# skypilot-org/skypilot

Hardware: AMD Instinct MI355X
Metric: tokens/sec (node) sky-launched Llama-3-8B (higher is better)
Workload: dtype bf16; 1 GPU; model=llama3-8b, global_batch=6, seq_len=4096, parallelism=dp1, sky_launched=True

## Files before the change

### skypilot_amd/ops/csrc/attention_bwd.hip

```cpp
#include "attn_launch.h"
#include "common.h"

#define BM 64
#define BN 64

extern "C" __global__ void attn_bwd_pre_kernel(
    const unsigned short* __restrict__ dO, const unsigned short* __restrict__ O,
    float* __restrict__ Dvec, long long rows, int S, int Hq) {
  const int lane = threadIdx.x & 63;
  const long long wave_id =
      (long long)blockIdx.x * (blockDim.x >> 6) + (threadIdx.x >> 6);
  const long long stride = (long long)gridDim.x * (blockDim.x >> 6);
  for (long long row = wave_id; row < rows; row += stride) {
    const unsigned short* drow = dO + row * ATT_D;
    const unsigned short* orow = O + row * ATT_D;
    float acc = bf2f(drow[lane]) * bf2f(orow[lane]) +
                bf2f(drow[lane + 64]) * bf2f(orow[lane + 64]);
    acc = wave_reduce_sum(acc);
    const int hh = (int)(row % Hq);
    const long long bs = row / Hq;
    const int ss = (int)(bs % S);
    const long long bb = bs / S;
    if (lane == 0) Dvec[(bb * Hq + hh) * S + ss] = acc;
  }
// ... 219 lines not shown
      *(s16x8*)((char*)v_lds + swz(row * 256 + ch * 16, row)) = vv8;
#pragma unroll
      for (int j = 0; j < 8; ++j) {
        int d = ch * 8 + j;
        *(unsigned short*)((char*)kt_lds + swzT(d * 128 + row * 2, d)) =
            (unsigned short)kv8[j];
      }
    }
    __syncthreads();

    f32x4 st[4], dpt[4];
#pragma unroll
    for (int kv4 = 0; kv4 < 4; ++kv4) {
      st[kv4] = f32x4{0.f, 0.f, 0.f, 0.f};
      dpt[kv4] = f32x4{0.f, 0.f, 0.f, 0.f};
    }
#pragma unroll
    for (int ks = 0; ks < 4; ++ks)
#pragma unroll
      for (int kv4 = 0; kv4 < 4; ++kv4) {
        int krow = kv4 * 16 + lrow;
        s16x8 a_k = *(const s16x8*)((char*)k_lds +
            swz(krow * 256 + (ks * 32 + lgrp * 8) * 2, krow));
        st[kv4] = MFMA_BF16(as_bf16x8(a_k), as_bf16x8(q_b[ks]), st[kv4]);
        s16x8 a_v = *(const s16x8*)((char*)v_lds +
            swz(krow * 256 + (ks * 32 + lgrp * 8) * 2, krow));
        dpt[kv4] = MFMA_BF16(as_bf16x8(a_v), as_bf16x8(do_b[ks]),
                             dpt[kv4]);
      }

#pragma unroll
    for (int kv4 = 0; kv4 < 4; ++kv4)
#pragma unroll
      for (int r = 0; r < 4; ++r) {
        int kv = kvbase + kv4 * 16 + lgrp * 4 + r;
        float pv;
        if ((causal && kv > my_q) || my_lse == -INFINITY)
          pv = 0.f;
        else
          pv = __expf(st[kv4][r] * scale - my_lse);
        st[kv4][r] = pv * (dpt[kv4][r] - my_dvec);
      }

    s16x8 ds_b[2];
#pragma unroll
    for (int ks = 0; ks < 2; ++ks)
#pragma unroll
      for (int j = 0; j < 8; ++j) {
        int src = (2 * (lgrp & 1) + (j >> 2)) * 16 + lrow;
        float v0 = __shfl(st[2 * ks][j & 3], src, 64);
        float v1 = __shfl(st[2 * ks + 1][j & 3], src, 64);
        ds_b[ks][j] = (short)f2bf((lgrp >> 1) ? v1 : v0);
      }

#pragma unroll
    for (int ct = 0; ct < 8; ++ct)
#pragma unroll
      for (int ks = 0; ks < 2; ++ks) {
        int krow = ct * 16 + lrow;
        s16x8 a_kt = *(const s16x8*)((char*)kt_lds +
            swzT(krow * 128 + (ks * 32 + lgrp * 8) * 2, krow));
        dq_t[ct] = MFMA_BF16(as_bf16x8(a_kt), as_bf16x8(ds_b[ks]),
                             dq_t[ct]);
      }
  }

  unsigned short* dQb = dQ + ((long long)b * S * Hq + qh) * ATT_D;
  unsigned short* orow = dQb + (long long)my_q * q_rowstride;
#pragma unroll
  for (int ct = 0; ct < 8; ++ct) {
    s16x4 ov;
#pragma unroll
    for (int r = 0; r < 4; ++r)
      ov[r] = (short)f2bf(dq_t[ct][r] * scale);
    *(s16x4*)(orow + ct * 16 + lgrp * 4) = ov;
  }
}

extern "C" void attn_bwd_launch(const void* Q, const void* K, const void* V,
                                const void* O, const void* dO,
                                const float* lse, float* Dvec, void* dQ,
                                void* dK, void* dV, int B, int S, int Hq,
                                int Hkv, float scale, bool causal,
                                int dkv_variant, hipStream_t stream) {
  long long rows = (long long)B * S * Hq;
  hipLaunchKernelGGL(attn_bwd_pre_kernel, dim3(membound_grid(rows, 4)),
                     dim3(256), 0, stream, (const unsigned short*)dO,
                     (const unsigned short*)O, Dvec, rows, S, Hq);
  if (S % 128 == 0) {
    attn_bwd_v3_launch(Q, K, V, dO, lse, Dvec, dQ, dK, dV, B, S, Hq, Hkv,
                       scale, causal, dkv_variant, stream);
    return;
  }
  hipLaunchKernelGGL(attn_bwd_dkv_kernel, dim3(S / BN, B * Hkv), dim3(256),
                     0, stream, (const unsigned short*)Q,
                     (const unsigned short*)K, (const unsigned short*)V,
                     (const unsigned short*)dO, lse, Dvec,
                     (unsigned short*)dK, (unsigned short*)dV, B, S, Hq, Hkv,
                     scale, causal ? 1 : 0);
  hipLaunchKernelGGL(attn_bwd_dq_swapped_kernel, dim3(S / BM, B * Hq),
                     dim3(256), 0, stream, (const unsigned short*)Q,
                     (const unsigned short*)K, (const unsigned short*)V,
                     (const unsigned short*)dO, lse, Dvec,
                     (unsigned short*)dQ, B, S, Hq, Hkv, scale,
                     causal ? 1 : 0);
}
```

### skypilot_amd/ops/csrc/attention_bwd_v3.hip

```cpp
#include "attn_launch.h"
#include "attn_v3.h"

__device__ __forceinline__ int vsubz(int q, int d) {
  return (((q >> 2) << 3) + ((d >> 4) ^ ((q >> 2) & 7))) * 64 +
         ((q & 3) << 4) + (d & 15);
}

extern "C" __global__ __launch_bounds__(256, 2) void attn_bwd_dkv_v3_kernel(
    const unsigned short* __restrict__ Q, const unsigned short* __restrict__ K,
    const unsigned short* __restrict__ V, const unsigned short* __restrict__ dO,
    const float* __restrict__ lse, const float* __restrict__ Dvec,
    unsigned short* __restrict__ dK, unsigned short* __restrict__ dV, int B,
    int S, int Hq, int Hkv, float scale, int causal) {
  __shared__ unsigned short q_lds[32 * ATT_D];
  __shared__ unsigned short do_lds[32 * ATT_D];
  __shared__ unsigned short k_own[128 * ATT_D];
  __shared__ unsigned short v_own[128 * ATT_D];

  const int kt = blockIdx.x;
  const int bh = blockIdx.y;
  const int b = bh / Hkv;
  const int kvh = bh % Hkv;
  const int group = Hq / Hkv;
  const int kvb = kt * 128;
// ... 564 lines not shown
    for (int n = 0; n < 2; ++n)
#pragma unroll
      for (int r = 0; r < 16; ++r) {
        float p = exp2f(st[n][r] - lse2);
        dpt[n][r] = p * (dpt[n][r] - dvq);
      }

    tr4 t0, t1;
    s16x8 db;
#define DQ_TR_ISSUE(ks)                                                   \
  {                                                                       \
    unsigned base = (unsigned)(size_t)((char*)k_lds[buf]);                \
    int kv_s = (ks) * 16 + ((g >> 1) << 3) + (lw >> 2);                   \
    int d_s0 = ((g & 1) << 4) + ((lw & 3) << 2);                          \
    unsigned a0 = (unsigned)(kv_s * 256 +                                 \
                             ((((d_s0) >> 3) ^ (kv_s & 15)) << 4) +       \
                             ((d_s0 & 7) << 1));                          \
    unsigned a1 = (unsigned)((kv_s + 4) * 256 +                           \
                             ((((d_s0) >> 3) ^ ((kv_s + 4) & 15)) << 4) + \
                             ((d_s0 & 7) << 1));                          \
    unsigned a2 = (unsigned)(kv_s * 256 +                                 \
                             ((((32 + d_s0) >> 3) ^ (kv_s & 15)) << 4) +  \
                             ((d_s0 & 7) << 1));                          \
    unsigned a3 = (unsigned)((kv_s + 4) * 256 +                           \
                             ((((32 + d_s0) >> 3) ^ ((kv_s + 4) & 15))    \
                              << 4) +                                     \
                             ((d_s0 & 7) << 1));                          \
    ds_tr4_issue(&t0, base + a0, base + a1, base + a2, base + a3);        \
    unsigned a4 = (unsigned)(kv_s * 256 +                                 \
                             ((((64 + d_s0) >> 3) ^ (kv_s & 15)) << 4) +  \
                             ((d_s0 & 7) << 1));                          \
    unsigned a5 = (unsigned)((kv_s + 4) * 256 +                           \
                             ((((64 + d_s0) >> 3) ^ ((kv_s + 4) & 15))    \
                              << 4) +                                     \
                             ((d_s0 & 7) << 1));                          \
    unsigned a6 = (unsigned)(kv_s * 256 +                                 \
                             ((((96 + d_s0) >> 3) ^ (kv_s & 15)) << 4) +  \
                             ((d_s0 & 7) << 1));                          \
    unsigned a7 = (unsigned)((kv_s + 4) * 256 +                           \
                             ((((96 + d_s0) >> 3) ^ ((kv_s + 4) & 15))    \
                              << 4) +                                     \
                             ((d_s0 & 7) << 1));                          \
    ds_tr4_issue(&t1, base + a4, base + a5, base + a6, base + a7);        \
  }
#define DQ_MFMA(bfrag)                                                    \
  {                                                                       \
    union { unsigned long long u[2]; s16x8 v; } af;                       \
    __builtin_amdgcn_s_setprio(1);                                        \
    af.u[0] = t0.d[0];                                                    \
    af.u[1] = t0.d[1];                                                    \
    dq_acc[0] = MFMA32V3(as_bf16x8(af.v), as_bf16x8(bfrag), dq_acc[0]);   \
    af.u[0] = t0.d[2];                                                    \
    af.u[1] = t0.d[3];                                                    \
    dq_acc[1] = MFMA32V3(as_bf16x8(af.v), as_bf16x8(bfrag), dq_acc[1]);   \
    af.u[0] = t1.d[0];                                                    \
    af.u[1] = t1.d[1];                                                    \
    dq_acc[2] = MFMA32V3(as_bf16x8(af.v), as_bf16x8(bfrag), dq_acc[2]);   \
    af.u[0] = t1.d[2];                                                    \
    af.u[1] = t1.d[3];                                                    \
    dq_acc[3] = MFMA32V3(as_bf16x8(af.v), as_bf16x8(bfrag), dq_acc[3]);   \
    __builtin_amdgcn_s_setprio(0);                                        \
  }
    DQ_TR_ISSUE(0);
    V3_PACK2(db, dpt, 0);
    lgkm_wait0_bind2(&t0, &t1);
    DQ_MFMA(db);
    DQ_TR_ISSUE(1);
    V3_PACK2(db, dpt, 1);
    lgkm_wait0_bind2(&t0, &t1);
    DQ_MFMA(db);
    DQ_TR_ISSUE(2);
    V3_PACK2(db, dpt, 2);
    lgkm_wait0_bind2(&t0, &t1);
    DQ_MFMA(db);
    DQ_TR_ISSUE(3);
    V3_PACK2(db, dpt, 3);
    lgkm_wait0_bind2(&t0, &t1);
    DQ_MFMA(db);
  }

  DQ_EPILOGUE();
#undef DQ_EPILOGUE
#undef DQ_LOAD_Q
}

extern "C" void attn_bwd_v3_launch(const void* Q, const void* K,
                                   const void* V, const void* dO,
                                   const float* lse, const float* Dvec,
                                   void* dQ, void* dK, void* dV, int B,
                                   int S, int Hq, int Hkv, float scale,
                                   bool causal, int dkv_variant,
                                   hipStream_t stream) {
  const int variant = dkv_variant >= 0 ? dkv_variant : 2;
  if (variant == 0) {
    dim3 gkv(S / 128, B * Hkv);
    hipLaunchKernelGGL(attn_bwd_dkv_v3_kernel, gkv, dim3(256), 0, stream,
                       (const unsigned short*)Q, (const unsigned short*)K,
                       (const unsigned short*)V, (const unsigned short*)dO,
                       lse, Dvec, (unsigned short*)dK, (unsigned short*)dV,
                       B, S, Hq, Hkv, scale, causal ? 1 : 0);
  } else {
    const int heavy_first = variant == 2 ? 1 : 0;
    dim3 gkv = heavy_first ? dim3(B * Hkv, S / 128) : dim3(S / 128, B * Hkv);
    hipLaunchKernelGGL(attn_bwd_dkv_v3p_kernel, gkv, dim3(256), 0, stream,
                       (const unsigned short*)Q, (const unsigned short*)K,
                       (const unsigned short*)V, (const unsigned short*)dO,
                       lse, Dvec, (unsigned short*)dK, (unsigned short*)dV,
                       B, S, Hq, Hkv, scale, causal ? 1 : 0, heavy_first);
  }
  int nqq = S / 128;
  int gqx = (causal && nqq % 2 == 0) ? nqq / 2 : nqq;
  dim3 gq(gqx, B * Hq);
  hipLaunchKernelGGL(attn_bwd_dq_v3_kernel, gq, dim3(256), 0, stream,
                     (const unsigned short*)Q, (const unsigned short*)K,
                     (const unsigned short*)V, (const unsigned short*)dO,
                     lse, Dvec, (unsigned short*)dQ, B, S, Hq, Hkv, scale,
                     causal ? 1 : 0);
}
```

### skypilot_amd/ops/csrc/attn_launch.h

```cpp
#pragma once

#include <hip/hip_runtime.h>

#define ATT_D 128

extern "C" {
void attn_fwd_launch(const void* Q, const void* K, const void* V, void* O,
                     float* lse, int B, int S, int Hq, int Hkv, float scale,
                     bool causal, hipStream_t stream);
void attn_bwd_launch(const void* Q, const void* K, const void* V,
                     const void* O, const void* dO, const float* lse,
                     float* Dvec, void* dQ, void* dK, void* dV, int B, int S,
                     int Hq, int Hkv, float scale, bool causal,
                     int dkv_variant, hipStream_t stream);

void attn_fwd_v3_launch(const void* Q, const void* K, const void* V, void* O,
                        float* lse, int B, int S, int Hq, int Hkv,
                        float scale, bool causal, hipStream_t stream);
void attn_bwd_v3_launch(const void* Q, const void* K, const void* V,
                        const void* dO, const float* lse, const float* Dvec,
                        void* dQ, void* dK, void* dV, int B, int S, int Hq,
                        int Hkv, float scale, bool causal, int dkv_variant,
                        hipStream_t stream);
}
```

### skypilot_amd/ops/csrc/attn_v3.h

```cpp
#pragma once
#include "common.h"

typedef __attribute__((ext_vector_type(16))) float f32x16;
#define MFMA32V3(a, b, c) \
  __builtin_amdgcn_mfma_f32_32x32x16_bf16(a, b, c, 0, 0, 0)

__device__ __forceinline__ int swzK16(int byte_off, int row) {
  return byte_off ^ ((row & 15) << 4);
}

__device__ __forceinline__ int vsub(int kv, int d) {
  return (((kv >> 2) << 3) + (d >> 4)) * 64 + ((kv & 3) << 4) + (d & 15);
}

__device__ __forceinline__ unsigned cvtpk_bf16(float a, float b) {
  unsigned r;
  asm volatile("v_cvt_pk_bf16_f32 %0, %1, %2" : "=v"(r) : "v"(a), "v"(b));
  return r;
}

__device__ __forceinline__ float xhalf32(float x) {
  union { float f; unsigned u; } c;
  c.f = x;
  auto p = __builtin_amdgcn_permlane32_swap(c.u, c.u, false, false);
  union { unsigned u; float f; } r0, r1;
  r0.u = p[0];
  r1.u = p[1];
  return (threadIdx.x & 32) ? r0.f : r1.f;
}

__device__ __forceinline__ void vm_drain() {
  asm volatile("s_waitcnt vmcnt(0)" ::: "memory");
}

__device__ __forceinline__ void lgkm_wait0_bind2(tr4* a, tr4* b) {
  asm volatile("s_waitcnt lgkmcnt(0)"
               : "+v"(a->d[0]), "+v"(a->d[1]), "+v"(a->d[2]),
                 "+v"(a->d[3]), "+v"(b->d[0]), "+v"(b->d[1]),
                 "+v"(b->d[2]), "+v"(b->d[3])
               :
               : "memory");
  __builtin_amdgcn_sched_barrier(0);
}

template <int OFF>
__device__ __forceinline__ void ds_tr4_issue_off(tr4* t, unsigned a0,
                                                 unsigned a1, unsigned a2,
                                                 unsigned a3) {
  static_assert(OFF >= 0 && OFF < 65536, "DS offset field is 16 bits");
  asm volatile(
      "ds_read_b64_tr_b16 %0, %4 offset:%8\n\t"
      "ds_read_b64_tr_b16 %1, %5 offset:%8\n\t"
      "ds_read_b64_tr_b16 %2, %6 offset:%8\n\t"
      "ds_read_b64_tr_b16 %3, %7 offset:%8"
      : "=v"(t->d[0]), "=v"(t->d[1]), "=v"(t->d[2]), "=v"(t->d[3])
      : "v"(a0), "v"(a1), "v"(a2), "v"(a3), "n"(OFF)
      : "memory");
}

__device__ __forceinline__ void gload_lds16(const void* g, void* l) {
  __builtin_amdgcn_global_load_lds(
      (const __attribute__((address_space(1))) unsigned int*)g,
      (__attribute__((address_space(3))) unsigned int*)l, 16, 0, 0);
}


#define V3_PACK_CORE(pb, c0, c1, c2, c3, c4, c5, c6, c7)                  \
  {                                                                       \
    unsigned w0a = cvtpk_bf16(c0, c1);                                    \
    unsigned w1a = cvtpk_bf16(c2, c3);                                    \
    unsigned w0b = cvtpk_bf16(c4, c5);                                    \
    unsigned w1b = cvtpk_bf16(c6, c7);                                    \
    auto p0 = __builtin_amdgcn_permlane32_swap(w0a, w0b, false, false);   \
    auto p1 = __builtin_amdgcn_permlane32_swap(w1a, w1b, false, false);   \
    union { unsigned u[4]; s16x8 v; } pk;                                 \
    pk.u[0] = p0[0];                                                      \
    pk.u[1] = p1[0];                                                      \
    pk.u[2] = p0[1];                                                      \
    pk.u[3] = p1[1];                                                      \
    pb = pk.v;                                                            \
  }
#define V3_PACK2(pb, stv, ks)                                             \
  {                                                                       \
    const int e0 = ((ks) & 1) << 3;                                       \
    const int n = (ks) >> 1;                                              \
    V3_PACK_CORE(pb, stv[n][e0 + 0], stv[n][e0 + 1], stv[n][e0 + 2],      \
                 stv[n][e0 + 3], stv[n][e0 + 4], stv[n][e0 + 5],          \
                 stv[n][e0 + 6], stv[n][e0 + 7]);                         \
  }
#define V3_PACK1(pb, stv, ks)                                             \
  {                                                                       \
    const int e0 = (ks) << 3;                                             \
    V3_PACK_CORE(pb, stv[e0 + 0], stv[e0 + 1], stv[e0 + 2],               \
                 stv[e0 + 3], stv[e0 + 4], stv[e0 + 5], stv[e0 + 6],      \
                 stv[e0 + 7]);                                            \
  }
```

### skypilot_amd/ops/csrc/bindings.cpp

```cpp
#include <torch/extension.h>

#include <ATen/hip/HIPContext.h>
#include <hip/hip_runtime.h>

#include <vector>

#include "attn_append.h"
#include "attn_launch.h"

#define CHECK_GPU(x) TORCH_CHECK(x.is_cuda(), #x " must be on GPU")
#define CHECK_CONTIG(x) TORCH_CHECK(x.is_contiguous(), #x " must be contiguous")
#define CHECK_BF16(x) \
  TORCH_CHECK(x.scalar_type() == at::kBFloat16, #x " must be bf16")

static hipStream_t cur_stream() {
  return at::hip::getCurrentHIPStream().stream();
}

extern "C" {
void rmsnorm_fwd_launch(const void*, const void*, void*, float*, long long,
                        int, float, hipStream_t);
void rmsnorm_bwd_launch(const void*, const void*, const void*, const float*,
                        void*, float*, long long, int, hipStream_t);
void rope_launch(const void*, void*, const float*, const float*, const int*,
// ... 117 lines not shown
              H, D, backward, cur_stream());
  return y;
}

void adamw_step(std::vector<torch::Tensor> params_bf16,
                std::vector<torch::Tensor> params_master,
                std::vector<torch::Tensor> grads,
                std::vector<torch::Tensor> exp_avg,
                std::vector<torch::Tensor> exp_avg_sq, double lr, double beta1,
                double beta2, double eps, double weight_decay, int64_t step,
                double grad_scale, std::vector<bool> decay_mask) {
  auto stream = cur_stream();
  for (size_t i = 0; i < params_bf16.size(); ++i) {
    auto& p = params_bf16[i];
    long long n = p.numel();
    float wd = decay_mask.empty() || decay_mask[i] ? (float)weight_decay : 0.f;
    adamw_launch(p.data_ptr(), params_master[i].data_ptr<float>(),
                 grads[i].data_ptr(), exp_avg[i].data_ptr<float>(),
                 exp_avg_sq[i].data_ptr<float>(), n, (float)lr, (float)beta1,
                 (float)beta2, (float)eps, wd, (int)step, (float)grad_scale,
                 stream);
  }
}

torch::Tensor cross_entropy_fused(torch::Tensor logits, torch::Tensor targets,
                                  double grad_scale, int64_t ignore_index) {
  CHECK_GPU(logits); CHECK_CONTIG(logits); CHECK_BF16(logits);
  TORCH_CHECK(targets.scalar_type() == at::kInt);
  const int V = (int)logits.size(-1);
  long long N = logits.numel() / V;
  auto loss = torch::empty({(long)N}, logits.options().dtype(at::kFloat));
  cross_entropy_launch(logits.data_ptr(), targets.data_ptr<int>(),
                       loss.data_ptr<float>(), N, V, (float)grad_scale,
                       (int)ignore_index, cur_stream());
  return loss;
}

static void check_attn_qkv(const char* op, const torch::Tensor& Q,
                           const torch::Tensor& K, const torch::Tensor& V) {
  const torch::Tensor* ts[] = {&Q, &K, &V};
  const char* names[] = {"Q", "K", "V"};
  for (int i = 0; i < 3; ++i) {
    const torch::Tensor& t = *ts[i];
    TORCH_CHECK(t.is_cuda(), op, ": ", names[i], " must be on GPU");
    TORCH_CHECK(t.scalar_type() == at::kBFloat16, op, ": ", names[i],
                " must be bf16, got ", t.scalar_type());
    TORCH_CHECK(t.dim() == 4, op, ": ", names[i],
                " must be [B, S, heads, 128], got ", t.dim(), " dims");
    TORCH_CHECK(t.is_contiguous(), op, ": ", names[i],
                " must be contiguous, got strides ", t.strides());
    TORCH_CHECK(t.size(3) == ATT_D, op, ": ", names[i],
                " head dim must be 128, got ", t.size(3));
  }
  const int64_t B = Q.size(0), S = Q.size(1), Hq = Q.size(2);
  TORCH_CHECK(S % 64 == 0, op, ": seq len must be a multiple of 64, got ", S);
  TORCH_CHECK(K.size(0) == B && K.size(1) == S, op,
              ": K must be [B, S, Hkv, 128] with Q's B = ", B, " and S = ", S,
              ", got ", K.sizes());
  TORCH_CHECK(V.sizes() == K.sizes(), op, ": V must have K's shape ",
              K.sizes(), ", got ", V.sizes());
  const int64_t Hkv = K.size(2);
  TORCH_CHECK(Hkv > 0 && Hq % Hkv == 0, op, ": Hq = ", Hq,
              " must be a multiple of Hkv = ", Hkv);
}

std::vector<torch::Tensor> attn_fwd(torch::Tensor Q, torch::Tensor K,
                                    torch::Tensor V, double scale,
                                    bool causal) {
  check_attn_qkv("attn_fwd", Q, K, V);
  const int B = (int)Q.size(0), S = (int)Q.size(1), Hq = (int)Q.size(2);
  const int Hkv = (int)K.size(2);
  auto O = torch::empty_like(Q);
  auto lse = torch::empty({B, Hq, S}, Q.options().dtype(at::kFloat));
  attn_fwd_launch(Q.data_ptr(), K.data_ptr(), V.data_ptr(), O.data_ptr(),
                  lse.data_ptr<float>(), B, S, Hq, Hkv, (float)scale, causal,
                  cur_stream());
  return {O, lse};
}

std::vector<torch::Tensor> attn_bwd(torch::Tensor Q, torch::Tensor K,
                                    torch::Tensor V, torch::Tensor O,
                                    torch::Tensor dO, torch::Tensor lse,
                                    double scale, bool causal,
                                    int64_t dkv_variant) {
  check_attn_qkv("attn_bwd", Q, K, V);
  TORCH_CHECK(dkv_variant >= -1 && dkv_variant <= 2,
              "attn_bwd: dkv_variant must be -1, 0, 1 or 2");
  const int B = (int)Q.size(0), S = (int)Q.size(1), Hq = (int)Q.size(2);
  const int Hkv = (int)K.size(2);
  const torch::Tensor* outs[] = {&O, &dO};
  const char* out_names[] = {"O", "dO"};
  for (int i = 0; i < 2; ++i) {
    const torch::Tensor& t = *outs[i];
    TORCH_CHECK(t.is_cuda() && t.scalar_type() == at::kBFloat16, "attn_bwd: ",
                out_names[i], " must be bf16 on GPU, got ", t.scalar_type());
    TORCH_CHECK(t.sizes() == Q.sizes(), "attn_bwd: ", out_names[i],
                " must have Q's shape ", Q.sizes(), ", got ", t.sizes());
    TORCH_CHECK(t.is_contiguous(), "attn_bwd: ", out_names[i],
                " must be contiguous, got strides ", t.strides());
  }
  TORCH_CHECK(lse.is_cuda() && lse.scalar_type() == at::kFloat,
              "attn_bwd: lse must be fp32 on GPU, got ", lse.scalar_type());
  TORCH_CHECK(lse.dim() == 3 && lse.size(0) == B && lse.size(1) == Hq &&
                  lse.size(2) == S,
              "attn_bwd: lse must be [B, Hq, S] = [", B, ", ", Hq, ", ", S,
              "], got ", lse.sizes());
  TORCH_CHECK(lse.is_contiguous(),
              "attn_bwd: lse must be contiguous, got strides ", lse.strides());
  auto dQ = torch::empty_like(Q);
  auto dK = torch::empty_like(K);
  auto dV = torch::empty_like(V);
  auto Dvec = torch::empty({(long)B * S * Hq}, Q.options().dtype(at::kFloat));
  attn_bwd_launch(Q.data_ptr(), K.data_ptr(), V.data_ptr(), O.data_ptr(),
                  dO.data_ptr(), lse.data_ptr<float>(),
                  Dvec.data_ptr<float>(), dQ.data_ptr(), dK.data_ptr(),
                  dV.data_ptr(), B, S, Hq, Hkv, (float)scale, causal,
                  (int)dkv_variant, cur_stream());
  return {dQ, dK, dV};
}

torch::Tensor attn_decode(torch::Tensor Q, torch::Tensor Kc,
                          torch::Tensor Vc, torch::Tensor kv_lens,
                          torch::Tensor slot_ids, double scale) {
  CHECK_GPU(Q); CHECK_CONTIG(Q); CHECK_BF16(Q);
  TORCH_CHECK(kv_lens.scalar_type() == at::kInt);
  TORCH_CHECK(slot_ids.scalar_type() == at::kInt);
  const int B = (int)Q.size(0), Hq = (int)Q.size(1), D = (int)Q.size(2);
  const int S_max = (int)Kc.size(1), Hkv = (int)Kc.size(2);
  TORCH_CHECK(D == 128);
  auto O = torch::empty_like(Q);
  attn_decode_launch(Q.data_ptr(), Kc.data_ptr(), Vc.data_ptr(),
                     O.data_ptr(), kv_lens.data_ptr<int>(),
                     slot_ids.data_ptr<int>(), B, S_max, Hq,
                     Hkv, (float)scale, cur_stream());
  return O;
}

torch::Tensor attn_append(torch::Tensor Q, torch::Tensor Kc,
                          torch::Tensor Vc, torch::Tensor slot_ids,
                          torch::Tensor q_start, torch::Tensor q_lens,
                          double scale) {
  const char* op = "attn_append";
  const torch::Tensor* ts[] = {&Q, &Kc, &Vc};
  const char* names[] = {"Q", "Kc", "Vc"};
  for (int i = 0; i < 3; ++i) {
    const torch::Tensor& t = *ts[i];
    TORCH_CHECK(t.is_cuda(), op, ": ", names[i], " must be on GPU");
    TORCH_CHECK(t.scalar_type() == at::kBFloat16, op, ": ", names[i],
                " must be bf16, got ", t.scalar_type());
    TORCH_CHECK(t.dim() == 4, op, ": ", names[i],
                " must have 4 dims [.., .., heads, 128], got ", t.dim());
    TORCH_CHECK(t.is_contiguous(), op, ": ", names[i],
                " must be contiguous, got strides ", t.strides());
    TORCH_CHECK(t.size(3) == ATT_D, op, ": ", names[i],
                " head dim must be 128, got ", t.size(3));
  }
  const int64_t n = Q.size(0), Sq = Q.size(1), Hq = Q.size(2);
  const int64_t slots = Kc.size(0), S_max = Kc.size(1), Hkv = Kc.size(2);
  TORCH_CHECK(Sq > 0 && Sq % 64 == 0, op,
              ": chunk length Sq must be a positive multiple of 64, got ",
              Sq);
  TORCH_CHECK(Vc.sizes() == Kc.sizes(), op, ": Vc must have Kc's shape ",
              Kc.sizes(), ", got ", Vc.sizes());
  TORCH_CHECK(slots > 0 && S_max > 0, op,
              ": the cache must hold at least one slot and one row, got ",
              Kc.sizes());
  TORCH_CHECK(Hkv > 0 && Hq % Hkv == 0, op, ": Hq = ", Hq,
              " must be a multiple of Hkv = ", Hkv);
  TORCH_CHECK(n > 0 && n * Hq <= 65535, op, ": n * Hq = ", n * Hq,
              " must be in [1, 65535] (one grid row per sequence and head)");
  TORCH_CHECK(Q.device() == Kc.device() && Q.device() == Vc.device(), op,
              ": Q, Kc and Vc must be on one device");
  const torch::Tensor* idx[] = {&slot_ids, &q_start, &q_lens};
  const char* idx_names[] = {"slot_ids", "q_start", "q_lens"};
  for (int i = 0; i < 3; ++i) {
    const torch::Tensor& t = *idx[i];
    TORCH_CHECK(t.is_cuda() && t.device() == Q.device(), op, ": ",
                idx_names[i], " must be on Q's GPU");
    TORCH_CHECK(t.scalar_type() == at::kInt, op, ": ", idx_names[i],
                " must be int32, got ", t.scalar_type());
    TORCH_CHECK(t.dim() == 1 && t.size(0) == n && t.is_contiguous(), op,
                ": ", idx_names[i], " must be a contiguous [n] = [", n,
                "] tensor, got ", t.sizes());
  }
  auto O = torch::empty_like(Q);
  attn_append_launch(Q.data_ptr(), Kc.data_ptr(), Vc.data_ptr(),
                     O.data_ptr(), slot_ids.data_ptr<int>(),
                     q_start.data_ptr<int>(), q_lens.data_ptr<int>(), (int)n,
                     (int)Sq, (int)Hq, (int)Hkv, (int)slots, (int)S_max,
                     (float)scale, cur_stream());
  return O;
}

torch::Tensor attn_decode_qkv(torch::Tensor qkv, torch::Tensor Kc,
                              torch::Tensor Vc, torch::Tensor cos_tab,
                              torch::Tensor sin_tab,
                              torch::Tensor positions,
                              torch::Tensor kv_lens,
                              torch::Tensor slot_ids, int64_t Hq,
                              int64_t Hkv, double scale) {
// ... 244 lines not shown
  TORCH_CHECK(qkv.size(1) == (Hq + 2 * Hkv) * D,
              "rope_kvwrite: packed width mismatch");
  auto q = torch::empty({n, (long)Hq, (long)D}, qkv.options());
  rope_kvwrite_launch(qkv.data_ptr(), q.data_ptr(), kc.data_ptr(),
                      vc.data_ptr(), cos_tab.data_ptr(),
                      sin_tab.data_ptr(), positions.data_ptr(),
                      slot_ids.data_ptr(), n, (int)Hq, (int)Hkv, D, S_max,
                      cur_stream());
  return q;
}

torch::Tensor swiglu_fwd(torch::Tensor gu) {
  CHECK_GPU(gu); CHECK_CONTIG(gu); CHECK_BF16(gu);
  const int M2 = (int)gu.size(-1);
  TORCH_CHECK(M2 % 16 == 0, "swiglu_fwd: last dim must be 2*M with "
              "M % 8 == 0, got ", M2);
  long long rows = gu.numel() / M2;
  auto sizes = gu.sizes().vec();
  sizes.back() = M2 / 2;
  auto y = torch::empty(sizes, gu.options());
  swiglu_fwd_launch(gu.data_ptr(), y.data_ptr(), rows, M2 / 2,
                    cur_stream());
  return y;
}

torch::Tensor swiglu_bwd(torch::Tensor gu, torch::Tensor dy) {
  CHECK_GPU(gu); CHECK_CONTIG(gu); CHECK_BF16(gu);
  CHECK_GPU(dy); CHECK_CONTIG(dy); CHECK_BF16(dy);
  const int M2 = (int)gu.size(-1);
  TORCH_CHECK(M2 % 16 == 0, "swiglu_bwd: last dim must be 2*M with "
              "M % 8 == 0, got ", M2);
  auto ysizes = gu.sizes().vec();
  ysizes.back() = M2 / 2;
  TORCH_CHECK(dy.sizes() == at::IntArrayRef(ysizes),
              "swiglu_bwd: dy must have the shape of swiglu_fwd(gu)");
  long long rows = gu.numel() / M2;
  auto dgu = torch::empty_like(gu);
  swiglu_bwd_launch(gu.data_ptr(), dy.data_ptr(), dgu.data_ptr(), rows,
                    M2 / 2, cur_stream());
  return dgu;
}

torch::Tensor mfma_probe(torch::Tensor A, torch::Tensor B) {
  CHECK_GPU(A); CHECK_BF16(A); CHECK_CONTIG(A); CHECK_CONTIG(B);
  TORCH_CHECK(A.size(0) == 16 && A.size(1) == 32);
  TORCH_CHECK(B.size(0) == 32 && B.size(1) == 16);
  auto C = torch::zeros({16, 16}, A.options().dtype(at::kFloat));
  mfma_probe_launch(A.data_ptr(), B.data_ptr(), C.data_ptr<float>(),
                    cur_stream());
  return C;
}

torch::Tensor mfma32_probe(torch::Tensor A, torch::Tensor B) {
  CHECK_GPU(A); CHECK_BF16(A); CHECK_CONTIG(A); CHECK_CONTIG(B);
  TORCH_CHECK(A.size(0) == 32 && A.size(1) == 16);
  TORCH_CHECK(B.size(0) == 16 && B.size(1) == 32);
  auto C = torch::zeros({32, 32}, A.options().dtype(at::kFloat));
  mfma32_probe_launch(A.data_ptr(), B.data_ptr(), C.data_ptr<float>(),
                      cur_stream());
  return C;
}

torch::Tensor trb16_probe(int64_t mode, torch::Tensor ref_dev) {
  auto out = torch::zeros({64, 4}, ref_dev.options().dtype(at::kFloat));
  trb16_probe_launch(out.data_ptr<float>(), (int)mode, cur_stream());
  return out;
}

torch::Tensor permlane_probe(torch::Tensor ref_dev) {
  auto out = torch::zeros({64, 2}, ref_dev.options().dtype(at::kFloat));
  permlane_probe_launch(out.data_ptr<float>(), cur_stream());
  return out;
}

PYBIND11_MODULE(TORCH_EXTENSION_NAME, m) {
  m.def("rmsnorm_fwd", &rmsnorm_fwd);
  m.def("rmsnorm_bwd", &rmsnorm_bwd);
  m.def("rope", &rope);
  m.def("adamw_step", &adamw_step);
  m.def("cross_entropy_fused", &cross_entropy_fused);
  m.def("attn_fwd", &attn_fwd);
  m.def("attn_bwd", &attn_bwd, py::arg("Q"), py::arg("K"), py::arg("V"),
        py::arg("O"), py::arg("dO"), py::arg("lse"), py::arg("scale"),
        py::arg("causal"), py::arg("dkv_variant") = -1);
  m.def("attn_decode", &attn_decode);
  m.def("attn_append", &attn_append);
  m.def("skinny_gemm", &skinny_gemm);
  m.def("skinny_gemm_fp8", &skinny_gemm_fp8);
  m.def("transpose_bf16", &transpose_bf16);
  m.def("gemm_nt", &gemm_nt);
  m.def("wgrad_tn", &wgrad_tn);
  m.def("adamw_step_mt", &adamw_step_mt);
  m.def("skinny_gemm_swiglu", &skinny_gemm_swiglu);
  m.def("rmsnorm_res", &rmsnorm_res);
  m.def("rope_kvwrite", &rope_kvwrite);
  m.def("decode_advance", &decode_advance);
  m.def("sample_tokens", &sample_tokens);
  m.def("decode_sample_advance", &decode_sample_advance);
  m.def("attn_decode_qkv", &attn_decode_qkv);
  m.def("skinny_gemm_fp8_norm", &skinny_gemm_fp8_norm);
  m.def("swiglu_fwd", &swiglu_fwd);
  m.def("swiglu_bwd", &swiglu_bwd);
  m.def("mfma_probe", &mfma_probe);
  m.def("mfma32_probe", &mfma32_probe);
  m.def("trb16_probe", &trb16_probe);
  m.def("permlane_probe", &permlane_probe);
}
```

Baseline: 20680 tokens/s.

## Add pipelined dQ backward kernel with double-buffered async K/V staging

Adds a new dQ backward attention kernel that stages K/V tiles into LDS with direct global-to-LDS loads in a double buffer, overlapping the next tile's load with the current tile's MFMAs. LDS reads are interleaved with MFMA steps using immediate-offset reads and fine-grained lgkmcnt waits. Causal q-tiles are paired per block for load balance. The new kernel becomes the default through a dq_variant switch, and the old kernel stays selectable. This costs more LDS per block and carries risk in the hand-written waitcnt scheduling.

```diff
diff --git a/skypilot_amd/ops/csrc/attention_bwd.hip b/skypilot_amd/ops/csrc/attention_bwd.hip
--- a/skypilot_amd/ops/csrc/attention_bwd.hip
+++ b/skypilot_amd/ops/csrc/attention_bwd.hip
@@ -325,14 +325,15 @@
                                 const float* lse, float* Dvec, void* dQ,
                                 void* dK, void* dV, int B, int S, int Hq,
                                 int Hkv, float scale, bool causal,
-                                int dkv_variant, hipStream_t stream) {
+                                int dkv_variant, int dq_variant,
+                                hipStream_t stream) {
   long long rows = (long long)B * S * Hq;
   hipLaunchKernelGGL(attn_bwd_pre_kernel, dim3(membound_grid(rows, 4)),
                      dim3(256), 0, stream, (const unsigned short*)dO,
                      (const unsigned short*)O, Dvec, rows, S, Hq);
   if (S % 128 == 0) {
     attn_bwd_v3_launch(Q, K, V, dO, lse, Dvec, dQ, dK, dV, B, S, Hq, Hkv,
-                       scale, causal, dkv_variant, stream);
+                       scale, causal, dkv_variant, dq_variant, stream);
     return;
   }
   hipLaunchKernelGGL(attn_bwd_dkv_kernel, dim3(S / BN, B * Hkv), dim3(256),
diff --git a/skypilot_amd/ops/csrc/attention_bwd_v3.hip b/skypilot_amd/ops/csrc/attention_bwd_v3.hip
--- a/skypilot_amd/ops/csrc/attention_bwd_v3.hip
+++ b/skypilot_amd/ops/csrc/attention_bwd_v3.hip
@@ -670,6 +670,250 @@
   DQ_EPILOGUE();
 #undef DQ_EPILOGUE
 #undef DQ_LOAD_Q
+#undef DQ_STAGE
+#undef DQ_TR_ISSUE
+}
+
+extern "C" __global__ __launch_bounds__(256, 2) void attn_bwd_dq_v3p_kernel(
+    const unsigned short* __restrict__ Q, const unsigned short* __restrict__ K,
+    const unsigned short* __restrict__ V, const unsigned short* __restrict__ dO,
+    const float* __restrict__ lse, const float* __restrict__ Dvec,
+    unsigned short* __restrict__ dQ, int B, int S, int Hq, int Hkv,
+    float scale, int causal) {
+  __shared__ unsigned short lds[4 * 64 * ATT_D];
+
+  const int nq = S / 128;
+  const bool paired = causal && (int)gridDim.x * 2 == nq;
+  const int qtA = paired ? nq - 1 - (int)blockIdx.x
+                         : (int)gridDim.x - 1 - (int)blockIdx.x;
+  const int qtB = paired ? (int)blockIdx.x : 0;
+  const int bh = blockIdx.y;
+  const int b = bh / Hq;
+  const int qh = bh % Hq;
+  const int kvh = qh / (Hq / Hkv);
+  int qbase = qtA * 128;
+
+  const int tid = threadIdx.x;
+  const int lane = tid & 63;
+  const int w = tid >> 6;
+  const int col = lane & 31;
+  const int h = lane >> 5;
+  const int g = lane >> 4;
+  const int lw = lane & 15;
+
+  const long long q_rowstride = (long long)Hq * ATT_D;
+  const long long kv_rowstride = (long long)Hkv * ATT_D;
+  const unsigned short* Qb = Q + ((long long)b * S * Hq + qh) * ATT_D;
+  const unsigned short* Kb = K + ((long long)b * S * Hkv + kvh) * ATT_D;
+  const unsigned short* Vb = V + ((long long)b * S * Hkv + kvh) * ATT_D;
+  const unsigned short* dOb = dO + ((long long)b * S * Hq + qh) * ATT_D;
+  const float* lse_b = lse + ((long long)b * Hq + qh) * S;
+  const float* dvec_b = Dvec + ((long long)b * Hq + qh) * S;
+
+  int my_q = qbase + 32 * w + col;
+
+  s16x8 q_b[8], do_b[8];
+  float lse2, dvq;
+#define DQP_LOAD_Q()                                                      \
+  {                                                                       \
+    const float qs = scale * 1.44269504088896340736f;                     \
+    const unsigned short* src = Qb + (long long)my_q * q_rowstride;       \
+    const unsigned short* dsrc = dOb + (long long)my_q * q_rowstride;     \
+    _Pragma("unroll") for (int ks = 0; ks < 8; ++ks)                      \
+      do_b[ks] = *(const s16x8*)(dsrc + ks * 16 + h * 8);                 \
+    _Pragma("unroll") for (int ks = 0; ks < 8; ++ks) {                    \
+      s16x8 raw = *(const s16x8*)(src + ks * 16 + h * 8);                 \
+      _Pragma("unroll") for (int j = 0; j < 8; ++j)                       \
+        raw[j] = (short)f2bf(bf2f((unsigned short)raw[j]) * qs);          \
+      q_b[ks] = raw;                                                      \
+    }                                                                     \
+    float lv = lse_b[my_q];                                               \
+    lse2 = (lv == -INFINITY) ? 3.0e37f                                    \
+                             : lv * 1.44269504088896340736f;              \
+    dvq = dvec_b[my_q];                                                   \
+    _Pragma("unroll") for (int ks = 0; ks < 8; ++ks)                      \
+      asm volatile("" : "+v"(do_b[ks]));                                  \
+    asm volatile("" : "+v"(lse2), "+v"(dvq));                             \
+  }
+
+  f32x16 dq_acc[4];
+#pragma unroll
+  for (int dt = 0; dt < 4; ++dt)
+#pragma unroll
+    for (int r = 0; r < 16; ++r) dq_acc[dt][r] = 0.f;
+
+  const int nt_A = causal ? (qbase + 128) / 64 : S / 64;
+  const int nt_B = paired ? (qtB * 128 + 128) / 64 : 0;
+  const int total_t = nt_A + nt_B;
+  int w_tiles = causal ? ((qbase + 32 * w + 31) >> 6) + 1 : nt_A;
+
+#define DQP_EPILOGUE()                                                    \
+  {                                                                       \
+    unsigned short* dQb = dQ + ((long long)b * S * Hq + qh) * ATT_D;      \
+    unsigned short* qrow = dQb + (long long)my_q * q_rowstride;           \
+    _Pragma("unroll") for (int dt = 0; dt < 4; ++dt)                      \
+      _Pragma("unroll") for (int rq = 0; rq < 4; ++rq) {                  \
+        s16x4 ov;                                                         \
+        _Pragma("unroll") for (int r = 0; r < 4; ++r)                     \
+          ov[r] = (short)f2bf(dq_acc[dt][rq * 4 + r] * scale);            \
+        *(s16x4*)(qrow + dt * 32 + rq * 8 + h * 4) = ov;                  \
+      }                                                                   \
+  }
+
+  const unsigned kv_rs2 = (unsigned)kv_rowstride * 2u;
+  const unsigned sg_off =
+      (unsigned)(16 * w + g) * kv_rs2 + (unsigned)((lw ^ g) << 4);
+#define DQP_STAGE(kvrow0, bufi)                                           \
+  {                                                                       \
+    gptr_t ksrc = uniform_ptr(Kb + (long long)(kvrow0) * kv_rowstride);   \
+    gptr_t vsrc = uniform_ptr(Vb + (long long)(kvrow0) * kv_rowstride);   \
+    _Pragma("unroll") for (int i = 0; i < 4; ++i) {                       \
+      const unsigned off = (sg_off ^ (unsigned)(i << 6)) + 4u * i * kv_rs2; \
+      char* dst = (char*)lds + (bufi) * 16384 + (16 * w + 4 * i) * 256;   \
+      gload_lds16(ksrc + off, dst);                                       \
+      gload_lds16(vsrc + off, dst + 32768);                               \
+    }                                                                     \
+  }
+
+  unsigned tra[8];
+  {
+    const int kv_s = ((g >> 1) << 3) + (lw >> 2);
+    const int d_s0 = ((g & 1) << 4) + ((lw & 3) << 2);
+    const unsigned base = (unsigned)(size_t)((char*)lds) + 16384u;
+#pragma unroll
+    for (int i = 0; i < 8; ++i) {
+      const int kv = kv_s + 4 * (i & 1);
+      const int d = 32 * (i >> 1) + d_s0;
+      tra[i] = base + (unsigned)(kv * 256 + (((d >> 3) ^ (kv & 15)) << 4) +
+                                 ((d & 7) << 1));
+    }
+  }
+  unsigned frag = (unsigned)swzK16(col * 256 + h * 16, col) + 16384u;
+
+  DQP_LOAD_Q();
+  DQP_STAGE(0, 0);
+
+  for (int it = 0; it < total_t; ++it) {
+    if (paired && it == nt_A) {
+      DQP_EPILOGUE();
+      qbase = qtB * 128;
+      my_q = qbase + 32 * w + col;
+      DQP_LOAD_Q();
+#pragma unroll
+      for (int dt = 0; dt < 4; ++dt)
+#pragma unroll
+        for (int r = 0; r < 16; ++r) dq_acc[dt][r] = 0.f;
+      w_tiles = ((qbase + 32 * w + 31) >> 6) + 1;
+    }
+    const int kt = it < nt_A ? it : it - nt_A;
+    const int buf = it & 1;
+    {
+      const unsigned flip = buf ? 16384u : (unsigned)-16384;
+      frag += flip;
+#pragma unroll
+      for (int i = 0; i < 8; ++i) tra[i] += flip;
+    }
+    vm_drain();
+    __syncthreads();
+    {
+      const int nx = it + 1 < total_t ? it + 1 : it;
+      const int kt2 = nx < nt_A ? nx : nx - nt_A;
+      DQP_STAGE(kt2 * 64, buf ^ 1);
+    }
+    if (kt >= w_tiles) continue;
+
+    const int kvbase = kt * 64;
+    f32x16 st[2], dpt[2];
+#pragma unroll
+    for (int n = 0; n < 2; ++n)
+#pragma unroll
+      for (int r = 0; r < 16; ++r) {
+        st[n][r] = 0.f;
+        dpt[n][r] = 0.f;
+      }
+    unsigned fr = frag;
+    asm volatile("" : "+v"(fr));
+    s16x8 fa[4];
+#define DQP_RD(i)                                                         \
+  ds_read128_issue_off<(((i) >> 1) & 1) * 8192 + ((i) & 1) * 32768>(      \
+      &fa[(i) & 3], fr ^ (unsigned)(((i) >> 2) << 5))
+#define DQP_STEP(i)                                                       \
+  {                                                                       \
+    lgkm_wait_bind1<((i) < 28 ? 3 : 31 - (i))>(&fa[(i) & 3]);             \
+    if ((i) & 1)                                                          \
+      dpt[((i) >> 1) & 1] =                                               \
+          MFMA32V3(as_bf16x8(fa[(i) & 3]), as_bf16x8(do_b[(i) >> 2]),     \
+                   dpt[((i) >> 1) & 1]);                                  \
+    else                                                                  \
+      st[((i) >> 1) & 1] =                                                \
+          MFMA32V3(as_bf16x8(fa[(i) & 3]), as_bf16x8(q_b[(i) >> 2]),      \
+                   st[((i) >> 1) & 1]);                                   \
+    __builtin_amdgcn_sched_barrier(0);                                    \
+    if ((i) + 4 < 32) DQP_RD((i) + 4);                                    \
+  }
+#define DQP_STEP4(i)                                                      \
+  DQP_STEP(i) DQP_STEP((i) + 1) DQP_STEP((i) + 2) DQP_STEP((i) + 3)
+    __builtin_amdgcn_s_setprio(1);
+    DQP_RD(0);
+    DQP_RD(1);
+    DQP_RD(2);
+    DQP_RD(3);
+    DQP_STEP4(0) DQP_STEP4(4) DQP_STEP4(8) DQP_STEP4(12)
+    DQP_STEP4(16) DQP_STEP4(20) DQP_STEP4(24) DQP_STEP4(28)
+    __builtin_amdgcn_s_setprio(0);
+#undef DQP_STEP4
+#undef DQP_STEP
+#undef DQP_RD
+
+    if (causal && kvbase + 63 > qbase + 32 * w) {
+#pragma unroll
+      for (int n = 0; n < 2; ++n)
+#pragma unroll
+        for (int r = 0; r < 16; ++r) {
+          int kv = kvbase + n * 32 + (r & 3) + ((r >> 2) << 3) + (h << 2);
+          if (kv > my_q) st[n][r] = -30000.f;
+        }
+    }
+#pragma unroll
+    for (int n = 0; n < 2; ++n)
+#pragma unroll
+      for (int r = 0; r < 16; ++r) {
+        float p = exp2f(st[n][r] - lse2);
+        dpt[n][r] = p * (dpt[n][r] - dvq);
+      }
+
+    tr4 t0, t1;
+    s16x8 db;
+#define DQP_TR_ISSUE(ks)                                                  \
+  {                                                                       \
+    ds_tr4_issue_off_ec<(ks) * 4096>(&t0, tra[0], tra[1], tra[2], tra[3]); \
+    ds_tr4_issue_off_ec<(ks) * 4096>(&t1, tra[4], tra[5], tra[6], tra[7]); \
+  }
+    DQP_TR_ISSUE(0);
+    V3_PACK2(db, dpt, 0);
+    lgkm_wait0_bind2(&t0, &t1);
+    DQ_MFMA(db);
+    DQP_TR_ISSUE(1);
+    V3_PACK2(db, dpt, 1);
+    lgkm_wait0_bind2(&t0, &t1);
+    DQ_MFMA(db);
+    DQP_TR_ISSUE(2);
+    V3_PACK2(db, dpt, 2);
+    lgkm_wait0_bind2(&t0, &t1);
+    DQ_MFMA(db);
+    DQP_TR_ISSUE(3);
+    V3_PACK2(db, dpt, 3);
+    lgkm_wait0_bind2(&t0, &t1);
+    DQ_MFMA(db);
+  }
+  vm_drain();
+
+  DQP_EPILOGUE();
+#undef DQP_EPILOGUE
+#undef DQP_LOAD_Q
+#undef DQP_STAGE
+#undef DQP_TR_ISSUE
+#undef DQ_MFMA
 }
 
 extern "C" void attn_bwd_v3_launch(const void* Q, const void* K,
@@ -678,7 +922,7 @@
                                    void* dQ, void* dK, void* dV, int B,
                                    int S, int Hq, int Hkv, float scale,
                                    bool causal, int dkv_variant,
-                                   hipStream_t stream) {
+                                   int dq_variant, hipStream_t stream) {
   const int variant = dkv_variant >= 0 ? dkv_variant : 2;
   if (variant == 0) {
     dim3 gkv(S / 128, B * Hkv);
@@ -699,7 +943,9 @@
   int nqq = S / 128;
   int gqx = (causal && nqq % 2 == 0) ? nqq / 2 : nqq;
   dim3 gq(gqx, B * Hq);
-  hipLaunchKernelGGL(attn_bwd_dq_v3_kernel, gq, dim3(256), 0, stream,
+  const int dqv = dq_variant >= 0 ? dq_variant : 1;
+  hipLaunchKernelGGL(dqv == 1 ? attn_bwd_dq_v3p_kernel : attn_bwd_dq_v3_kernel,
+                     gq, dim3(256), 0, stream,
                      (const unsigned short*)Q, (const unsigned short*)K,
                      (const unsigned short*)V, (const unsigned short*)dO,
                      lse, Dvec, (unsigned short*)dQ, B, S, Hq, Hkv, scale,
diff --git a/skypilot_amd/ops/csrc/attn_launch.h b/skypilot_amd/ops/csrc/attn_launch.h
--- a/skypilot_amd/ops/csrc/attn_launch.h
+++ b/skypilot_amd/ops/csrc/attn_launch.h
@@ -12,7 +12,7 @@
                      const void* O, const void* dO, const float* lse,
                      float* Dvec, void* dQ, void* dK, void* dV, int B, int S,
                      int Hq, int Hkv, float scale, bool causal,
-                     int dkv_variant, hipStream_t stream);
+                     int dkv_variant, int dq_variant, hipStream_t stream);
 
 void attn_fwd_v3_launch(const void* Q, const void* K, const void* V, void* O,
                         float* lse, int B, int S, int Hq, int Hkv,
@@ -21,5 +21,5 @@
                         const void* dO, const float* lse, const float* Dvec,
                         void* dQ, void* dK, void* dV, int B, int S, int Hq,
                         int Hkv, float scale, bool causal, int dkv_variant,
-                        hipStream_t stream);
+                        int dq_variant, hipStream_t stream);
 }
diff --git a/skypilot_amd/ops/csrc/attn_v3.h b/skypilot_amd/ops/csrc/attn_v3.h
--- a/skypilot_amd/ops/csrc/attn_v3.h
+++ b/skypilot_amd/ops/csrc/attn_v3.h
@@ -58,7 +58,43 @@
       : "memory");
 }
 
+template <int OFF>
+__device__ __forceinline__ void ds_tr4_issue_off_ec(tr4* t, unsigned a0,
+                                                    unsigned a1, unsigned a2,
+                                                    unsigned a3) {
+  static_assert(OFF >= 0 && OFF < 65536, "DS offset field is 16 bits");
+  asm volatile(
+      "ds_read_b64_tr_b16 %0, %4 offset:%8\n\t"
+      "ds_read_b64_tr_b16 %1, %5 offset:%8\n\t"
+      "ds_read_b64_tr_b16 %2, %6 offset:%8\n\t"
+      "ds_read_b64_tr_b16 %3, %7 offset:%8"
+      : "=&v"(t->d[0]), "=&v"(t->d[1]), "=&v"(t->d[2]), "=&v"(t->d[3])
+      : "v"(a0), "v"(a1), "v"(a2), "v"(a3), "n"(OFF)
+      : "memory");
+}
+
+template <int OFF>
+__device__ __forceinline__ void ds_read128_issue_off(s16x8* d, unsigned a) {
+  static_assert(OFF >= 0 && OFF < 65536, "DS offset field is 16 bits");
+  asm volatile("ds_read_b128 %0, %1 offset:%2"
+               : "=&v"(*d)
+               : "v"(a), "n"(OFF)
+               : "memory");
+}
+template <int N>
+__device__ __forceinline__ void lgkm_wait_bind1(s16x8* d) {
+  static_assert(N >= 0 && N < 16, "lgkmcnt is 4 bits");
+  asm volatile("s_waitcnt lgkmcnt(%1)" : "+v"(*d) : "n"(N) : "memory");
+  __builtin_amdgcn_sched_barrier(0);
+}
+
 __device__ __forceinline__ void gload_lds16(const void* g, void* l) {
+  __builtin_amdgcn_global_load_lds(
+      (const __attribute__((address_space(1))) unsigned int*)g,
+      (__attribute__((address_space(3))) unsigned int*)l, 16, 0, 0);
+}
+__device__ __forceinline__ void gload_lds16(
+    const __attribute__((address_space(1))) char* g, void* l) {
   __builtin_amdgcn_global_load_lds(
       (const __attribute__((address_space(1))) unsigned int*)g,
       (__attribute__((address_space(3))) unsigned int*)l, 16, 0, 0);
diff --git a/skypilot_amd/ops/csrc/bindings.cpp b/skypilot_amd/ops/csrc/bindings.cpp
--- a/skypilot_amd/ops/csrc/bindings.cpp
+++ b/skypilot_amd/ops/csrc/bindings.cpp
@@ -223,10 +223,13 @@
                                     torch::Tensor V, torch::Tensor O,
                                     torch::Tensor dO, torch::Tensor lse,
                                     double scale, bool causal,
-                                    int64_t dkv_variant) {
+                                    int64_t dkv_variant,
+                                    int64_t dq_variant) {
   check_attn_qkv("attn_bwd", Q, K, V);
   TORCH_CHECK(dkv_variant >= -1 && dkv_variant <= 2,
               "attn_bwd: dkv_variant must be -1, 0, 1 or 2");
+  TORCH_CHECK(dq_variant >= -1 && dq_variant <= 1,
+              "attn_bwd: dq_variant must be -1, 0 or 1");
   const int B = (int)Q.size(0), S = (int)Q.size(1), Hq = (int)Q.size(2);
   const int Hkv = (int)K.size(2);
   const torch::Tensor* outs[] = {&O, &dO};
@@ -256,7 +259,7 @@
                   dO.data_ptr(), lse.data_ptr<float>(),
                   Dvec.data_ptr<float>(), dQ.data_ptr(), dK.data_ptr(),
                   dV.data_ptr(), B, S, Hq, Hkv, (float)scale, causal,
-                  (int)dkv_variant, cur_stream());
+                  (int)dkv_variant, (int)dq_variant, cur_stream());
   return {dQ, dK, dV};
 }
 
@@ -667,7 +670,8 @@
   m.def("attn_fwd", &attn_fwd);
   m.def("attn_bwd", &attn_bwd, py::arg("Q"), py::arg("K"), py::arg("V"),
         py::arg("O"), py::arg("dO"), py::arg("lse"), py::arg("scale"),
-        py::arg("causal"), py::arg("dkv_variant") = -1);
+        py::arg("causal"), py::arg("dkv_variant") = -1,
+        py::arg("dq_variant") = -1);
   m.def("attn_decode", &attn_decode);
   m.def("attn_append", &attn_append);
   m.def("skinny_gemm", &skinny_gemm);
```

Measured after the change: 21400 tokens/s (median of 6 runs). 3.5% higher.
